# magneano/shyft

Measured on AMD Instinct MI355X. Metric: cell-steps/sec (cells×timesteps/wall) for pt_gs_k at 1/2/4/8 MI355X, higher is better.
Workload: dtype f64

## Files before the change

include/shyft_hip.h:

```cpp
#ifndef SHYFT_HIP_H
#define SHYFT_HIP_H

#include <stddef.h>
#include <stdint.h>

#ifdef __cplusplus
extern "C" {
#endif

typedef struct shyft_hip_region shyft_hip_region;

enum shyft_hip_stack {
    SHYFT_HIP_PT_GS_K = 1, SHYFT_HIP_HBV_STACK = 2, SHYFT_HIP_PT_SS_K = 3, SHYFT_HIP_PT_HS_K = 4, SHYFT_HIP_PT_HPS_K = 5
};

enum shyft_hip_forcing {
    SHYFT_HIP_TEMPERATURE = 0, SHYFT_HIP_PRECIPITATION = 1, SHYFT_HIP_WIND_SPEED = 2,
    SHYFT_HIP_REL_HUM = 3, SHYFT_HIP_RADIATION = 4
};

enum shyft_hip_collect { SHYFT_HIP_COLLECT_DISCHARGE = 0, SHYFT_HIP_COLLECT_DISCHARGE_SNOW = 1, SHYFT_HIP_COLLECT_ALL = 2 };

enum shyft_hip_ptgsk_series {
    SHYFT_HIP_AVG_DISCHARGE = 0, SHYFT_HIP_CHARGE_M3S = 1, SHYFT_HIP_SNOW_SCA = 2, SHYFT_HIP_SNOW_SWE = 3,
// ... 83 lines not shown
                         int weighted, size_t step0, size_t n, double* dst);
int shyft_hip_catchment_sums(const shyft_hip_region* h, int series, size_t step0, size_t n, double* dst,
                             int dst_on_device);
int shyft_hip_catchment_area_sums(const shyft_hip_region* h, int series, size_t step0, size_t n, double* dst,
                                  int dst_on_device);

#define SHYFT_HIP_PERCENTILES_MAX 16
#define SHYFT_HIP_PERCENTILES_LDS_MAX 4096
enum shyft_hip_statistics_property {
    SHYFT_HIP_STAT_AVERAGE = -1, SHYFT_HIP_STAT_MIN_EXTREME = -1000, SHYFT_HIP_STAT_MAX_EXTREME = 1000
};
int shyft_hip_percentiles(const shyft_hip_region* h, int series, const int64_t* ids, size_t n_ids, int scope,
                          const int64_t* pct, size_t n_pct, size_t step0, size_t n, double* dst);
int shyft_hip_catchment_percentiles(const shyft_hip_region* h, int series, const int64_t* pct, size_t n_pct,
                                    size_t step0, size_t n, double* dst, int dst_on_device);
int shyft_hip_percentiles_host(const double* rows, size_t n_steps, size_t n_samples_per_step, const int64_t* pct,
                               size_t n_pct, double* dst);
enum shyft_hip_percentiles_path_id {
    SHYFT_HIP_PERCENTILES_NONE = 0, SHYFT_HIP_PERCENTILES_LDS_SORT = 1, SHYFT_HIP_PERCENTILES_RADIX = 2
};
int shyft_hip_percentiles_path(const shyft_hip_region* h);
double shyft_hip_last_percentiles_ms(const shyft_hip_region* h);

int shyft_hip_kalman_run(int device, int n, size_t M, size_t T, const double* bias, const int32_t* fold, const double* w,
                         double v2, int mode, double* x, double* k, double* P, double* out, int save_every,
                         const int32_t* piece_begin, const int32_t* piece_ix, const double* piece_seconds);
int shyft_hip_kalman_run_host(int n, size_t M, size_t T, const double* bias, const int32_t* fold, const double* w, double v2,
                              int mode, double* x, double* k, double* P, double* out, int save_every,
                              const int32_t* piece_begin, const int32_t* piece_ix, const double* piece_seconds);
int shyft_hip_kalman_initial_state(int n, double covariance_init, double hourly_correlation, double process_noise_init,
                                   double* P, double* W);
double shyft_hip_kalman_last_ms(int device);

#define SHYFT_HIP_QM_MAX_SERIES 1024
#define SHYFT_HIP_QM_PRIOR 0
#define SHYFT_HIP_QM_QM 1
#define SHYFT_HIP_QM_BLEND 2
int shyft_hip_quantile_map(int device, size_t B, size_t T, size_t F, size_t P, const double* fc, const double* w,
                           const double* pri, const int32_t* mode, const double* interp_weight,
                           int interpolated_quantiles, double* out);
int shyft_hip_quantile_map_host(size_t B, size_t T, size_t F, size_t P, const double* fc, const double* w,
                                const double* pri, const int32_t* mode, const double* interp_weight,
                                int interpolated_quantiles, double* out);
#define SHYFT_HIP_QM_PATH_NONE 0
#define SHYFT_HIP_QM_PATH_WAVE 1
#define SHYFT_HIP_QM_PATH_GROUP 2
int shyft_hip_quantile_map_last_path(int device);
double shyft_hip_quantile_map_last_ms(int device);

#define SHYFT_HIP_RESAMPLE_AVERAGE 0
#define SHYFT_HIP_RESAMPLE_INTEGRAL 1
#define SHYFT_HIP_RESAMPLE_ACCUMULATE 2
int shyft_hip_resample(int device, int mode, size_t S, const int64_t* row, const int64_t* t, const double* v,
                       const int64_t* t_end, const int32_t* fx, int64_t ta_t0, int64_t ta_dt, size_t T, double* out);
int shyft_hip_resample_host(int device, int mode, size_t S, const int64_t* row, const int64_t* t, const double* v,
                            const int64_t* t_end, const int32_t* fx, int64_t ta_t0, int64_t ta_dt, size_t T,
                            double* out);
double shyft_hip_resample_last_ms(int device);
uint64_t shyft_hip_resample_calls(int device);
#define SHYFT_HIP_RESAMPLE_PATH_AUTO 0
#define SHYFT_HIP_RESAMPLE_PATH_DIRECT 1
#define SHYFT_HIP_RESAMPLE_PATH_TILED 2
int shyft_hip_resample_set_path(int path);
int shyft_hip_resample_last_path(int device);

int shyft_hip_ts_rating_curve(int device, size_t S, const int64_t* row, const int64_t* t, const double* v,
                              const int64_t* t_end, const int32_t* fx, size_t P, const int64_t* pack_row,
                              const int64_t* curve_t, const int64_t* curve_row, const double* seg, const int64_t* pack_of,
                              double* out);
int shyft_hip_ts_rating_curve_host(int device, size_t S, const int64_t* row, const int64_t* t, const double* v,
                                   const int64_t* t_end, const int32_t* fx, size_t P, const int64_t* pack_row,
                                   const int64_t* curve_t, const int64_t* curve_row, const double* seg,
                                   const int64_t* pack_of, double* out);
int shyft_hip_ts_ice_packing(int device, size_t S, const int64_t* row, const int64_t* t, const double* v,
                             const int64_t* t_end, const int32_t* fx, const int64_t* qrow, const int64_t* qt,
                             const int64_t* window, const double* threshold, const int32_t* policy, double* out);
int shyft_hip_ts_ice_packing_host(int device, size_t S, const int64_t* row, const int64_t* t, const double* v,
                                  const int64_t* t_end, const int32_t* fx, const int64_t* qrow, const int64_t* qt,
                                  const int64_t* window, const double* threshold, const int32_t* policy, double* out);
int shyft_hip_ts_ice_packing_recession(int device, size_t S, const int64_t* row, const int64_t* t, const double* v,
                                       const int64_t* t_end, const int32_t* fx, const double* ice,
                                       const int64_t* ice_start, const int64_t* ice_end, const double* alpha,
                                       const double* recession_minimum, double* out);
int shyft_hip_ts_ice_packing_recession_host(int device, size_t S, const int64_t* row, const int64_t* t, const double* v,
                                            const int64_t* t_end, const int32_t* fx, const double* ice,
                                            const int64_t* ice_start, const int64_t* ice_end, const double* alpha,
                                            const double* recession_minimum, double* out);
int shyft_hip_ts_min_max_fill(int device, size_t S, const int64_t* row, const int64_t* t, const double* v,
                              const int64_t* t_end, const int32_t* fx, const double* min_x, const double* max_x,
                              const int64_t* max_timespan, double* out);
int shyft_hip_ts_min_max_fill_host(int device, size_t S, const int64_t* row, const int64_t* t, const double* v,
                                   const int64_t* t_end, const int32_t* fx, const double* min_x, const double* max_x,
                                   const int64_t* max_timespan, double* out);
double shyft_hip_tsprep_last_ms(int device);
uint64_t shyft_hip_tsprep_calls(int device);

int shyft_hip_forecast_skill(int device, size_t S, const int64_t* row, const int64_t* t, const double* v,
                             const int64_t* t_end, const int32_t* fx, size_t P, const int64_t* fc_row,
                             const int64_t* fc_ix, const int64_t* obs_ix, const int64_t* t0_offset, const int64_t* dt,
                             const int64_t* n, double* ns, double* sim, double* obs);
int shyft_hip_forecast_skill_host(int device, size_t S, const int64_t* row, const int64_t* t, const double* v,
                                  const int64_t* t_end, const int32_t* fx, size_t P, const int64_t* fc_row,
                                  const int64_t* fc_ix, const int64_t* obs_ix, const int64_t* t0_offset,
                                  const int64_t* dt, const int64_t* n, double* ns, double* sim, double* obs);
double shyft_hip_forecast_skill_last_ms(int device);
uint64_t shyft_hip_forecast_skill_calls(int device);

size_t shyft_hip_number_of_catchments(const shyft_hip_region* h);
int shyft_hip_catchment_ids(const shyft_hip_region* h, int64_t* cids);

int shyft_hip_region_clone(const shyft_hip_region* src, shyft_hip_region** out);

int shyft_hip_cell_series(shyft_hip_region* h, int series, size_t cell, size_t step0, size_t n, double* buf, int write);
int shyft_hip_sample_cells(const shyft_hip_region* h, int series, const int64_t* cells, size_t n_cells, size_t step0,
                           size_t n, double* dst);

enum shyft_hip_knob {
    SHYFT_HIP_KNOB_PTGSK_INSTANCE = 1, SHYFT_HIP_KNOB_BRENT_READ_DELAY = 2,
    SHYFT_HIP_KNOB_SERIAL_SHARDS = 3,
    SHYFT_HIP_KNOB_CLONE_FAIL_AT = 4,
    SHYFT_HIP_KNOB_PERCENTILES_PATH = 5
};
int shyft_hip_set_test_knob(shyft_hip_region* h, int knob, int64_t value);

int shyft_hip_forcing_ok(const shyft_hip_region* h, int* ok);


int shyft_hip_set_routing_groups(shyft_hip_region* h, const int32_t* group_of_cell, size_t n_groups);
int shyft_hip_routing_group_sums(const shyft_hip_region* h, size_t step0, size_t n, double* dst, int dst_on_device);
int shyft_hip_route(int device, size_t n_groups, size_t T, const double* group_sums, int src_on_device,
                    const double* group_uhg, const int32_t* group_len, const int32_t* group_river, size_t n_rivers,
                    const double* river_uhg, const int32_t* river_len, const int32_t* river_downstream, size_t max_len,
                    double* local, double* upstream, double* output, int dst_on_device);

int shyft_hip_ensemble_run(shyft_hip_region* h, const double* params, size_t n_members, size_t n_per_set,
                           int start_step, int n_steps, int collect);
int shyft_hip_ensemble_sums(const shyft_hip_region* h, int series, int area_weighted, size_t step0, size_t n,
                            double* dst, int dst_on_device);
double shyft_hip_ensemble_last_ms(const shyft_hip_region* h);

int shyft_hip_math_selftest(int fn, const double* x, const double* y, size_t n, double* out);

#define SHYFT_HIP_DST_EXPLOG_INLINE 0
#define SHYFT_HIP_DST_EXPLOG_CALLS 1
#define SHYFT_HIP_DST_EXPLOG_TABLE 2
#define SHYFT_HIP_DST_POWERS 3
#define SHYFT_HIP_DST_GAMMA_LEAN 4
#define SHYFT_HIP_DST_BRENT 5
#define SHYFT_HIP_DST_BRENT_SPEC4 6
#define SHYFT_HIP_DST_BRENT_SPEC2 7
#define SHYFT_HIP_DST_SKAUGEN 8
#define SHYFT_HIP_DST_SKAUGEN_GROUP2 9
#define SHYFT_HIP_DST_SKAUGEN_GROUP4 10
int shyft_hip_device_selftest(int fn, const double* in, size_t n_in_cols, size_t n, double* out, size_t n_out_cols);

#ifdef __cplusplus
}
#endif
#endif
```

shyft_amd/csrc/device/gs_brent.h:

```cpp
#pragma once
#include <hip/hip_runtime.h>

#include "ptgsk_dev.h"
#include "gamma_lean.h"

namespace shyft_dev {

__device__ __forceinline__ double gsb_calc_q(double a, double b, double z, double lga, double eps, double ap1,
                                             const gsb_k& k, bool& ok) {
    const gamma_p_result g = gsb_gamma_pq(a, z / b, lga, eps, ap1, k, ok);
    return a * b * g.p1 + z * (1.0 - g.p);
}

__device__ __noinline__ double gs_calc_q_general(double a, double b, double z, double lga) {
    return gs_calc_q(a, b, z, lga);
}

struct gsb_f {
    double a2, b2, lga2, Q1, eps, ap1;
    bool a_ok;
    gsb_k k;
    __device__ __forceinline__ gsb_f(double z1, double a1, double b1, double a2_, double b2_, double q1, double lga2_)
        : a2(a2_), b2(b2_), lga2(lga2_) {
        Q1 = q1 == q1 ? q1 : gs_calc_q_general(a1, b1, z1, dlgamma(a1));
        k = gsb_load();
        eps = detmath::gamma_snow_policy_eps(a2);
        ap1 = a2 + 1.0;
        a_ok = a2 > 0.0;
    }
    __device__ __forceinline__ double operator()(double z) const {
        bool ok;
        double cq = gsb_calc_q(a2, b2, z, lga2, eps, ap1, k, ok);
        if (!(ok && a_ok)) cq = gs_calc_q_general(a2, b2, z, lga2);
        const double v = cq - Q1;
        return v * v;
    }
};

__device__ __forceinline__ double gs_brent_point(double z1, int k) {
    const double tolerance = 0x1p-11;
    const double golden = (double)0.3819660f;
    auto golden_step = [&](double x, double lo, double hi) {
        const double mid = (lo + hi) / 2;
        const double fract1 = tolerance * fabs(x) + tolerance / 4;
        const double d2 = (x >= mid) ? lo - x : hi - x;
        const double delta = golden * d2;
        return (fabs(delta) >= fract1) ? (x + delta) : (delta > 0 ? x + fabs(fract1) : x - fabs(fract1));
    };
    if (k == 0) return z1;
    const double u1 = golden_step(z1, 0.0, z1);
    if (k == 1) return u1;
    double lo = 0.0, hi = z1, x = z1;
    if (k == 2) {
        if (u1 >= x) lo = x; else hi = x;
        x = u1;
    } else {
        if (u1 < x) lo = u1; else hi = u1;
    }
    return golden_step(x, lo, hi);
}

struct gsb_zf {
    double z, f;
};
__device__ __noinline__ gsb_zf gs_corr_lwc_spec(double z1, double a1, double b1, double a2, double b2, double q1,
                                                double lga2, int k) {
    const gsb_f f(z1, a1, b1, a2, b2, q1, lga2);
    gsb_zf r;
    r.z = gs_brent_point(z1, k);
    r.f = f(r.z);
    return r;
}

struct gsb_memo {
    double z[4], f[4];
};

template <bool MEMO>
__device__ __forceinline__ double gs_corr_lwc_lean_t(double z1, double a1, double b1, double a2, double b2, double q1,
                                                     double lga2, const gsb_memo* memo) {
#ifdef SHYFT_ABLATE_BRENT
    return z1 * 0.5;
#endif
    const gsb_f fe(z1, a1, b1, a2, b2, q1, lga2);
    gsb_memo mm;
    if (MEMO) mm = *memo;
    auto f = [&](double z) {
        if (MEMO) {
            const long long zb = __double_as_longlong(z);
            bool hit = false;
            double r = 0.0;
#pragma unroll
            for (int i = 0; i < 4; ++i)
                if (!hit && zb == __double_as_longlong(mm.z[i])) { hit = true; r = mm.f[i]; }
            if (hit) return r;
        }
        return fe(z);
    };
    double min = 0.0, max = z1;
    const double tolerance = 0x1p-11;
    const double golden = (double)0.3819660f;
    double x, w, v, u, delta, delta2, fu, fv, fw, fx, mid, fract1, fract2;
    x = w = v = max;
    fw = fv = fx = f(x);
    delta2 = delta = 0;
    int count = 60;
    do {
        mid = (min + max) / 2;
        fract1 = tolerance * fabs(x) + tolerance / 4;
        fract2 = 2 * fract1;
        if (fabs(x - mid) <= (fract2 - (max - min) / 2)) break;
        if (fabs(delta2) > fract1) {
            double r = (x - w) * (fx - fv);
            double q = (x - v) * (fx - fw);
            double p = (x - v) * q - (x - w) * r;
            q = 2 * (q - r);
            if (q > 0) p = -p;
            q = fabs(q);
            double td = delta2;
            delta2 = delta;
            if ((fabs(p) >= fabs(q * td / 2)) || (p <= q * (min - x)) || (p >= q * (max - x))) {
                delta2 = (x >= mid) ? min - x : max - x;
                delta = golden * delta2;
            } else {
                delta = p / q;
                u = x + delta;
                if (((u - min) < fract2) || ((max - u) < fract2)) delta = (mid - x) < 0 ? -fabs(fract1) : fabs(fract1);
            }
        } else {
            delta2 = (x >= mid) ? min - x : max - x;
            delta = golden * delta2;
        }
        u = (fabs(delta) >= fract1) ? (x + delta) : (delta > 0 ? x + fabs(fract1) : x - fabs(fract1));
        fu = f(u);
        if (fu <= fx) {
            if (u >= x) min = x; else max = x;
            v = w; w = x; x = u;
            fv = fw; fw = fx; fx = fu;
        } else {
            if (u < x) min = u; else max = u;
            if ((fu <= fw) || (w == x)) {
                v = w; w = u; fv = fw; fw = fu;
            } else if ((fu <= fv) || (v == x) || (v == w)) {
                v = u; fv = fu;
            }
        }
    } while (--count);
    return x;
}

__device__ __noinline__ double gs_corr_lwc_lean(double z1, double a1, double b1, double a2, double b2, double q1,
                                                double lga2) {
    return gs_corr_lwc_lean_t<false>(z1, a1, b1, a2, b2, q1, lga2, nullptr);
}

__device__ __noinline__ double gs_corr_lwc_memo(double z1, double a1, double b1, double a2, double b2, double q1,
                                                double lga2, const gsb_memo& memo) {
    return gs_corr_lwc_lean_t<true>(z1, a1, b1, a2, b2, q1, lga2, &memo);
}

}
```

shyft_amd/csrc/kernels/ptgsk.hip:

```cpp
#include <hip/hip_runtime.h>
#include <stdint.h>
#include <stdlib.h>

#include "../device/ptgsk_dev.h"
#include "../device/gs_brent.h"
#include "../device/stream.h"
#include "../device/wave_place.h"
#include "../include_internal/kernels.h"
#include "../../../include/shyft_hip.h"

using namespace shyft_dev;

#define GS_BRENT_JOB gs_corr_lwc_lean

#ifdef SHYFT_PROF
__device__ unsigned long long g_ptgsk_prof[12];
extern "C" int shyft_ptgsk_prof_read(unsigned long long* out) {
    if (hipMemcpyFromSymbol(out, HIP_SYMBOL(g_ptgsk_prof), sizeof(g_ptgsk_prof)) != hipSuccess) return 1;
    unsigned long long z[12] = {};
    return hipMemcpyToSymbol(HIP_SYMBOL(g_ptgsk_prof), z, sizeof z) != hipSuccess;
}
#define PROF_DECL unsigned long long prof_acc[6] = {0, 0, 0, 0, 0, 0}, prof_lg = 0; unsigned long long prof_t = __builtin_amdgcn_s_memtime();
#define PROF_MARK(k) do { const unsigned long long t_ = __builtin_amdgcn_s_memtime(); prof_acc[k] += t_ - prof_t; prof_t = t_; } while (0)
#define PROF_FLUSH() do { if ((threadIdx.x & 63) == 0) { for (int k_ = 0; k_ < 6; ++k_) atomicAdd(&g_ptgsk_prof[k_], prof_acc[k_]); atomicAdd(&g_ptgsk_prof[11], prof_lg); } } while (0)
#else
#define PROF_DECL
#define PROF_MARK(k) ((void)0)
#define PROF_FLUSH() ((void)0)
#endif

namespace {

#ifndef SHYFT_PTGSK_NT
#define SHYFT_PTGSK_NT 1
#endif
constexpr bool STREAM_NT = SHYFT_PTGSK_NT != 0;

constexpr int BLOCK = 256;

#ifndef SHYFT_LB_WAVES
#define SHYFT_LB_WAVES 4
#endif

#ifndef SHYFT_PTGSK_LEAN
#define SHYFT_PTGSK_LEAN 1
#endif

constexpr int BRENT_PRIO = 3;

#ifndef SHYFT_PTGSK_LGQ
#define SHYFT_PTGSK_LGQ 1
#endif
#ifndef SHYFT_PTGSK_LGQ_NOBRENT
#define SHYFT_PTGSK_LGQ_NOBRENT 0
#endif
#ifndef SHYFT_PTGSK_LGQ_JOBLG
#define SHYFT_PTGSK_LGQ_JOBLG 1
#endif

template <bool COMPACT, bool UNIFORM, bool ENS = false, int WAVES = SHYFT_LB_WAVES, int B = BLOCK, bool SPEC = false,
          bool LEAN = false>
__global__ __launch_bounds__(B, WAVES) void ptgsk_run_kernel(const ptgsk_kargs a) {
    static_assert(COMPACT, "the Brent jobs always go through the workgroup queue");
    const int cell = blockIdx.x * blockDim.x + threadIdx.x;
    bool valid = cell < a.n_cells;
    if (valid && a.active && !a.active[cell]) valid = false;
    const int lc = valid ? cell : 0;
    const size_t N = (size_t)a.n_cells;
    const size_t NF = ENS ? (size_t)a.f_cols : N;
    const size_t fcl = ENS ? (size_t)a.fcol[lc] : (size_t)lc;
    const double* __restrict__ Pg = UNIFORM ? a.params : a.params + (size_t)a.set_ix[lc] * PTGSK_NP;
    __shared__ double lpar[UNIFORM ? PTGSK_NP : 1];
    if (UNIFORM && threadIdx.x < PTGSK_NP) lpar[threadIdx.x] = a.params[threadIdx.x];
    const double* __restrict__ P = UNIFORM ? (const double*)lpar : Pg;

    const double* __restrict__ cc = a.cellc;
    gs_cell gcell;
    gcell.forest_fraction = cc[PC_FOREST * N + lc];
    gcell.altitude = cc[PC_ALTITUDE * N + lc];
    gcell.cv2 = cc[PC_CV2 * N + lc];
    gcell.inv_cv2 = cc[PC_INV_CV2 * N + lc];
    __shared__ double lcc[11][B];
    {
        const int t = threadIdx.x;
        lcc[0][t] = gcell.forest_fraction;
        lcc[1][t] = gcell.altitude;
        lcc[2][t] = gcell.cv2;
        lcc[3][t] = gcell.inv_cv2;
        lcc[4][t] = cc[PC_GLACIER * N + lc];
        lcc[5][t] = cc[PC_SNOW_STORAGE * N + lc];
        lcc[6][t] = cc[PC_KIRCHNER_ROUTED_PREC * N + lc];
        lcc[7][t] = cc[PC_DIRECT_RESPONSE * N + lc];
        lcc[8][t] = cc[PC_AREA * N + lc];
    }
#define glacier_fraction (lcc[4][threadIdx.x])
#define snow_storage_fraction (lcc[5][threadIdx.x])
#define kirchner_routed_prec (lcc[6][threadIdx.x])
#define direct_response_fraction (lcc[7][threadIdx.x])
#define kirchner_fraction (1 - lcc[7][threadIdx.x])
#define cell_area_m2 (lcc[8][threadIdx.x])
#define glacier_area_m2 (lcc[8][threadIdx.x] * lcc[4][threadIdx.x])
#define LOAD_GCELL()                                   \
    do {                                               \
        gcell.forest_fraction = lcc[0][threadIdx.x];   \
        gcell.altitude = lcc[1][threadIdx.x];          \
        gcell.cv2 = lcc[2][threadIdx.x];               \
        gcell.inv_cv2 = lcc[3][threadIdx.x];           \
    } while (0)

    const double mmh_to_m3s_scale_factor = 1 / (3600.0 * 1000.0);

    double* __restrict__ st = a.state;
    gs_state s;
    s.albedo = st[PS_ALBEDO * N + lc];
    s.lwc = st[PS_LWC * N + lc];
    s.surface_heat = st[PS_SURFACE_HEAT * N + lc];
    s.alpha = st[PS_ALPHA * N + lc];
    s.sdc_melt_mean = st[PS_SDC_MELT_MEAN * N + lc];
    s.acc_melt = st[PS_ACC_MELT * N + lc];
    s.iso_pot_energy = st[PS_ISO_POT_ENERGY * N + lc];
    s.temp_swe = st[PS_TEMP_SWE * N + lc];
    double q = st[PS_KIRCHNER_Q * N + lc];
    lcc[9][threadIdx.x] = -1.0;
    lcc[10][threadIdx.x] = 0.0;
    constexpr bool LGQ = SHYFT_PTGSK_LGQ != 0 && B == 256 && !SPEC;
    constexpr bool JOBLG = LGQ && SHYFT_PTGSK_LGQ_JOBLG != 0;
    lgamma_cache_lds<JOBLG> lgc{lcc[9], lcc[10]};
    gs_carry carry;
    int32_t err = 0;

    const size_t TW = (size_t)a.win_len;
    const double* __restrict__ f_temp = a.forcing + (size_t)FV_TEMPERATURE * TW * NF;
    const double* __restrict__ f_prec = a.forcing + (size_t)FV_PRECIPITATION * TW * NF;
    const double* __restrict__ f_ws = a.forcing + (size_t)FV_WIND_SPEED * TW * NF;
    const double* __restrict__ f_rh = a.forcing + (size_t)FV_REL_HUM * TW * NF;
    const double* __restrict__ f_rad = a.forcing + (size_t)FV_RADIATION * TW * NF;
    double* __restrict__ R = a.resp;
    const size_t RS = TW * N;
    double* __restrict__ SS = LEAN ? nullptr : a.state_series;
    const size_t SSS = (TW + 1) * N;
    const int wed = (int)Pg[PK_WED];
    const int64_t snow_lo = (int64_t)((int)(Pg[PK_WED] * 24) - (int)(Pg[PK_NWD] * 24)) * 3600000000LL;
    const int64_t snow_hi = (int64_t)(int)(Pg[PK_WED] * 24) * 3600000000LL;

    __shared__ double jz1[B], ja1[B], jb1[B], ja2[B], jb2[B], jq1[B], jlg2[B], jres[B];
    __shared__ double jsz[SPEC ? 64 : 1], jsf[SPEC ? 64 : 1];
    __shared__ int jcount[2];
    __shared__ unsigned short lq[LGQ ? B : 1];
    __shared__ unsigned short jown[JOBLG ? B : 1];
    __shared__ int lcount[2];
    __shared__ int wsimd[B / 64];
    publish_wave_simd(wsimd);
    if (COMPACT) {
        if (threadIdx.x == 0) {
            jcount[0] = jcount[1] = 0;
            if (LGQ) lcount[0] = lcount[1] = 0;
        }
        __syncthreads();
    }
    const int jrot = solver_lane0<B>(wsimd);

    auto collect_state = [&](size_t wi) {
        SS[0 * SSS + wi * N + cell] = cell_area_m2 * q * mmh_to_m3s_scale_factor;
        SS[1 * SSS + wi * N + cell] = s.albedo;
        SS[2 * SSS + wi * N + cell] = s.lwc * snow_storage_fraction;
        SS[3 * SSS + wi * N + cell] = s.surface_heat;
        SS[4 * SSS + wi * N + cell] = s.alpha;
        SS[5 * SSS + wi * N + cell] = s.sdc_melt_mean;
        SS[6 * SSS + wi * N + cell] = s.acc_melt;
        SS[7 * SSS + wi * N + cell] = s.iso_pot_energy;
        SS[8 * SSS + wi * N + cell] = s.temp_swe * snow_storage_fraction;
    };

    const int i_end = a.step0 + a.n_steps;
    PROF_DECL
    for (int i = a.step0; i < i_end; ++i) {
        const double gm_direct = P[PK_GM_DIRECT];
        const double gm_routed = 1 - gm_direct;
        const double dtf = P[PK_DTF];
        const double p_corr = P[PK_PCORR];
        const double kc1 = P[PK_C1], kc2 = P[PK_C2], kc3 = P[PK_C3];
        const size_t wi = (size_t)(i - a.win0);
        const size_t fo = wi * N + lc;
        const size_t ff = ENS ? wi * NF + fcl : fo;
        double temp = 0, rad = 0, rel_hum = 0, prec = 0, wind_speed = 0;
        if (valid) {
            temp = stream_ld<STREAM_NT && !ENS>(&f_temp[ff]);
            rad = stream_ld<STREAM_NT && !ENS>(&f_rad[ff]);
            rel_hum = stream_ld<STREAM_NT && !ENS>(&f_rh[ff]);
            prec = stream_ld<STREAM_NT && !ENS>(&f_prec[ff]) * p_corr;
            wind_speed = stream_ld<STREAM_NT && !ENS>(&f_ws[ff]);
            if (SS) collect_state(wi);
        }
        const bool start_melt = a.doy[i] == wed;
        const int64_t trel = a.t_rel_year_us[i];
        const bool snow_season = trel >= snow_lo && trel < snow_hi;

        gs_mid m;
        m.need = false;
        m.done = true;
        LOAD_GCELL();
        if (threadIdx.x == 0) {
            jcount[(i + 1) & 1] = 0;
            if (LGQ) lcount[(i + 1) & 1] = 0;
        }
        int slot = -1;
        bool queued = false;
        auto new_shape = [&](double shape) {
            if (LGQ && shape != lcc[9][threadIdx.x]) {
                lq[atomicAdd(&lcount[i & 1], 1)] = (unsigned short)threadIdx.x;
                lcc[9][threadIdx.x] = shape;
                queued = true;
            }
        };
        auto brent_jobs = [&](int first, int nj) {
            if (JOBLG)
                for (int j = first; j < nj; j += B) {
                    const double lga2 = dlgamma(ja2[j]);
                    jlg2[j] = lga2;
                    const int o = jown[j];
                    if (lcc[9][o] == ja2[j]) lcc[10][o] = lga2;
                }
            for (int j = first; j < nj; j += B)
                jres[j] = GS_BRENT_JOB(jz1[j], ja1[j], jb1[j], ja2[j], jb2[j], jq1[j], jlg2[j]);
        };
        auto lgamma_jobs = [&](int first, int stride, int nl) {
            for (int j = first; j < nl; j += stride) {
                const int o = lq[j];
                lcc[10][o] = dlgamma(lcc[9][o]);
            }
        };
        auto enqueue = [&](double z1, double a1, double b1, double a2, double b2, double q1, double lga2) {
            slot = atomicAdd(&jcount[i & 1], 1);
            jz1[slot] = z1; ja1[slot] = a1; jb1[slot] = b1; ja2[slot] = a2; jb2[slot] = b2;
            jq1[slot] = q1; jlg2[slot] = lga2;
            if (JOBLG) jown[slot] = (unsigned short)threadIdx.x;
        };
#ifndef SHYFT_ABLATE_SNOW
        if (valid)
            gs_front(s, m, start_melt, a.dt_s, a.dt_us, P, gcell, temp, rad, prec, wind_speed, rel_hum, lgc, carry, enqueue,
                     new_shape);
#endif
        PROF_MARK(0);
        double z = 0.0;
        {
            __syncthreads();
            PROF_MARK(1);
            const int nj = jcount[i & 1];
            const int nl = LGQ ? lcount[i & 1] : 0;
            auto lgamma_phase = [&](int t) {
                const int ns = (nj + 63) & ~63;
                if (ns >= B) lgamma_jobs(t, B, nl);
                else if (t >= ns) lgamma_jobs(t - ns, B - ns, nl);
            };
            if (nj > 0) {
#ifdef SHYFT_PROF
                const unsigned long long tb = __builtin_amdgcn_s_memtime();
                if (threadIdx.x < nj) __builtin_amdgcn_s_setprio(BRENT_PRIO);
                brent_jobs((int)threadIdx.x, nj);
                __builtin_amdgcn_s_setprio(0);
                if (threadIdx.x < nj && (threadIdx.x & 63) == 0)
                    atomicAdd(&g_ptgsk_prof[8], (unsigned long long)(__builtin_amdgcn_s_memtime() - tb));
                if (LGQ && nl > 0) {
                    const unsigned long long tl = __builtin_amdgcn_s_memtime();
                    lgamma_phase((int)threadIdx.x);
                    prof_lg += __builtin_amdgcn_s_memtime() - tl;
                }
#else
                const int t = SPEC ? (int)threadIdx.x : (int)((threadIdx.x - jrot) & (B - 1));
                if (t < nj) __builtin_amdgcn_s_setprio(BRENT_PRIO);
                const int L = SPEC ? (4 * nj <= 64 ? 4 : 2 * nj <= 64 ? 2 : 0) : 0;
                if (L) {
                    const int jj = L == 4 ? t >> 2 : t >> 1;
                    if (t < 64 && jj < nj) {
                        const gsb_zf r = gs_corr_lwc_spec(jz1[jj], ja1[jj], jb1[jj], ja2[jj], jb2[jj], jq1[jj], jlg2[jj], t & (L - 1));
                        jsz[t] = r.z;
                        jsf[t] = r.f;
                    }
                    __syncthreads();
                    if (t < nj) {
                        gsb_memo mm;
#pragma unroll
                        for (int k = 0; k < 4; ++k) {
                            const int e = L * t + (k < L ? k : 0);
                            mm.z[k] = jsz[e];
                            mm.f[k] = jsf[e];
                        }
                        jres[t] = gs_corr_lwc_memo(jz1[t], ja1[t], jb1[t], ja2[t], jb2[t], jq1[t], jlg2[t], mm);
                    }
                } else {
                    brent_jobs(t, nj);
                }
                __builtin_amdgcn_s_setprio(0);
                if (LGQ && nl > 0) lgamma_phase(t);
#endif
                __syncthreads();
                if (!LEAN && a.read_delay > 0 && (threadIdx.x >> 6) != 0)
                    for (int k = 0; k < a.read_delay; ++k) __builtin_amdgcn_s_sleep(127);
                if (slot >= 0) z = jres[slot];
            } else if (LGQ && SHYFT_PTGSK_LGQ_NOBRENT > 0 && nl >= SHYFT_PTGSK_LGQ_NOBRENT) {
                lgamma_jobs((int)threadIdx.x, B, nl);
                __syncthreads();
            } else if (LGQ && queued) {
                lcc[10][threadIdx.x] = dlgamma(lcc[9][threadIdx.x]);
            }
        }
        PROF_MARK(2);
        if (!valid) {
            carry = gs_carry();
            continue;
        }
        double gs_sca, gs_storage, gs_outflow;
        LOAD_GCELL();
#ifdef SHYFT_ABLATE_SNOW
        gs_sca = 0.0; gs_storage = 0.0; gs_outflow = prec + 0.0 * z;
#else
        gs_back(s, m, z, gs_sca, gs_storage, gs_outflow, snow_season, a.dt_us, P, gcell, prec, lgc, carry);
#endif
        PROF_MARK(3);

        const double sca_area = cell_area_m2 * gs_sca;
        double gm_melt_m3s = 0.0;
        if (!(glacier_area_m2 <= sca_area || temp <= 0.0))
            gm_melt_m3s = dtf * temp * (glacier_area_m2 - sca_area) * (0.001 / 86400.0);
        double ae_exp;
        const double pot_evap =
            pt_pot_evap_exp<true>(P[PK_PT_ALBEDO], P[PK_PT_ALPHA], temp, rad, rel_hum, -q * 3.0 / P[PK_AE_SCALE], ae_exp) *
            3600.0;
        const double ae = pot_evap * (1.0 - ae_exp) * (1.0 - smax(gs_sca, glacier_fraction));
        const double gm_mmh = gm_melt_m3s / (mmh_to_m3s_scale_factor * cell_area_m2);
        PROF_MARK(4);
        double q_avg;
        if (!kirchner_step<true>(q, q_avg, gs_outflow * snow_storage_fraction + prec * kirchner_routed_prec + gm_routed * gm_mmh,
                           ae, a.t1_hours, kc1, kc2, kc3))
            err = ERR_KIRCHNER_MAX_ITER;
        const double total_discharge = smax(0.0, prec - ae) * direct_response_fraction + gm_direct * gm_mmh +
                                       q_avg * kirchner_fraction;
        const double charge_m3s = +(cell_area_m2 * prec * mmh_to_m3s_scale_factor) -
                                  (cell_area_m2 * ae * mmh_to_m3s_scale_factor) + gm_melt_m3s -
                                  (cell_area_m2 * total_discharge * mmh_to_m3s_scale_factor);
        stream_st<STREAM_NT>(&R[0 * RS + fo], cell_area_m2 * total_discharge * mmh_to_m3s_scale_factor);
        stream_st<STREAM_NT>(&R[1 * RS + fo], charge_m3s);
        if (!LEAN && a.collect >= 1) {
            R[2 * RS + fo] = gs_sca;
            R[3 * RS + fo] = gs_storage * snow_storage_fraction;
        }
        if (!LEAN && a.collect >= 2) {
            R[4 * RS + fo] = cell_area_m2 * (gs_outflow * snow_storage_fraction) * mmh_to_m3s_scale_factor;
            R[5 * RS + fo] = gm_melt_m3s;
            R[6 * RS + fo] = ae;
            R[7 * RS + fo] = pot_evap;
        }
        if (SS && i + 1 == i_end) collect_state(wi + 1);
        PROF_MARK(5);
    }
    PROF_FLUSH();
    if (!valid) return;
    st[PS_ALBEDO * N + cell] = s.albedo;
    st[PS_LWC * N + cell] = s.lwc;
    st[PS_SURFACE_HEAT * N + cell] = s.surface_heat;
    st[PS_ALPHA * N + cell] = s.alpha;
    st[PS_SDC_MELT_MEAN * N + cell] = s.sdc_melt_mean;
    st[PS_ACC_MELT * N + cell] = s.acc_melt;
    st[PS_ISO_POT_ENERGY * N + cell] = s.iso_pot_energy;
    st[PS_TEMP_SWE * N + cell] = s.temp_swe;
    st[PS_KIRCHNER_Q * N + cell] = q;
    if (err) a.err[cell] = err;
}
#undef LOAD_GCELL
#undef glacier_fraction
#undef snow_storage_fraction
#undef kirchner_routed_prec
#undef direct_response_fraction
#undef kirchner_fraction
#undef cell_area_m2
#undef glacier_area_m2

#ifndef SHYFT_PTGSK_BUDGET_WAVES
#define SHYFT_PTGSK_BUDGET_WAVES 7
#endif
__global__ __launch_bounds__(256, SHYFT_PTGSK_BUDGET_WAVES) void ptgsk_callee_budget_kernel(const ptgsk_kargs a) {
    if (a.n_cells >= 0) return;
    const int c = threadIdx.x;
    gs_state s{};
    gs_mid m{};
    lgamma_cache lgc;
    gs_carry carry;
    gs_cell gc{};
    double q = a.dt_s, qa = 0.0, sca, sto, outf;
    double j[7] = {};
    gs_front(s, m, c == 0, a.dt_s, a.dt_us, a.params, gc, q, q, q, q, q, lgc, carry,
             [&](double z1, double a1, double b1, double a2, double b2, double q1, double lga2) {
                 j[0] = z1; j[1] = a1; j[2] = b1; j[3] = a2; j[4] = b2; j[5] = q1; j[6] = lga2;
             });
    const double z = gs_corr_lwc_lean(j[0], j[1], j[2], j[3], j[4], j[5], j[6]);
    gs_back(s, m, z, sca, sto, outf, c == 1, a.dt_us, a.params, gc, q, lgc, carry);
    double e;
    const double pe = pt_pot_evap_exp<true>(0.2, 1.26, q, q, q, q, e);
    kirchner_step<true>(q, qa, outf, pe * e, a.t1_hours, -2.4, 0.9, -0.1);
    a.resp[c] = q + qa + sca + sto + s.lwc;
}

constexpr int ST_BLOCK = 256;

__global__ __launch_bounds__(ST_BLOCK, SHYFT_PTGSK_BUDGET_WAVES) void ptgsk_st_explog_inline_kernel(
    const double* __restrict__ in, size_t n, double* __restrict__ out) {
    const size_t i = blockIdx.x * (size_t)ST_BLOCK + threadIdx.x;
    if (i >= n) return;
    const kmath<true> km;
    const double x = in[i];
    out[i] = km.exp(x);
    out[n + i] = km.log(x);
}

__global__ __launch_bounds__(ST_BLOCK, SHYFT_PTGSK_BUDGET_WAVES) void ptgsk_st_explog_calls_kernel(
    const double* __restrict__ in, size_t n, double* __restrict__ out) {
    const size_t i = blockIdx.x * (size_t)ST_BLOCK + threadIdx.x;
    if (i >= n) return;
    const double x = in[i], y = in[n + i];
    out[i] = dexp(x);
    out[n + i] = dlog(x);
    const dexp_pair e = dexp2(x, y);
    out[2 * n + i] = e.a;
    out[3 * n + i] = e.b;
}

__global__ __launch_bounds__(ST_BLOCK, SHYFT_PTGSK_BUDGET_WAVES) void ptgsk_st_powers_kernel(
    const double* __restrict__ in, size_t n, double* __restrict__ out) {
    const size_t i = blockIdx.x * (size_t)ST_BLOCK + threadIdx.x;
    if (i >= n) return;
    const double x = in[i], y = in[n + i];
    out[i] = dpowr(x, y);
    out[n + i] = dpow4(x);
    out[2 * n + i] = dpow8(x);
    out[3 * n + i] = dpow(x, y);
}

__global__ __launch_bounds__(ST_BLOCK, SHYFT_PTGSK_BUDGET_WAVES) void ptgsk_st_gamma_kernel(
    const double* __restrict__ in, size_t n, double* __restrict__ out) {
    const size_t i = blockIdx.x * (size_t)ST_BLOCK + threadIdx.x;
    if (i >= n) return;
    const double a = in[i], x = in[n + i];
    const double lga = dlgamma(a);
    bool ok;
    (void)gsb_gamma_pq(a, x, lga, detmath::gamma_snow_policy_eps(a), a + 1.0, gsb_load(), ok);
    const gamma_p_result r = gs_gamma_pq_cs(a, x, lga);
    out[i] = r.p;
    out[n + i] = r.p1;
    out[2 * n + i] = r.prefix;
    out[3 * n + i] = ok ? 1.0 : 0.0;
}

__device__ __forceinline__ double st_brent_q1(double mode, double z1, double a1, double b1) {
    return mode != 0.0 ? gs_calc_q(a1, b1, z1, dlgamma(a1)) : __builtin_nan("");
}

__global__ __launch_bounds__(ST_BLOCK, SHYFT_PTGSK_BUDGET_WAVES) void ptgsk_st_brent_kernel(
    const double* __restrict__ in, size_t n, double* __restrict__ out) {
    const size_t i = blockIdx.x * (size_t)ST_BLOCK + threadIdx.x;
    if (i >= n) return;
    const double z1 = in[i], a1 = in[n + i], b1 = in[2 * n + i], a2 = in[3 * n + i], b2 = in[4 * n + i];
    const double q1 = st_brent_q1(in[5 * n + i], z1, a1, b1);
    const double lga2 = dlgamma(a2);
#ifdef SHYFT_PROF
    int nf_evals = 0;
    out[i] = gs_corr_lwc(z1, a1, b1, a2, b2, q1, lga2, nf_evals);
#else
    out[i] = gs_corr_lwc(z1, a1, b1, a2, b2, q1, lga2);
#endif
    out[n + i] = GS_BRENT_JOB(z1, a1, b1, a2, b2, q1, lga2);
}

template <int L>
__global__ __launch_bounds__(64, 2) void ptgsk_st_brent_spec_kernel(const double* __restrict__ in, size_t n,
                                                                    double* __restrict__ out) {
    static_assert(L == 4 || L == 2, "4 or 2 point lanes per job");
    constexpr int JOBS = 64 / L;
    __shared__ double jz1[JOBS], ja1[JOBS], jb1[JOBS], ja2[JOBS], jb2[JOBS], jq1[JOBS], jlg2[JOBS];
    __shared__ double jsz[64], jsf[64];
    const int t = threadIdx.x;
    const size_t j0 = blockIdx.x * (size_t)JOBS;
    const int nj = n - j0 < (size_t)JOBS ? (int)(n - j0) : JOBS;
    if (t < nj) {
        const size_t i = j0 + t;
        jz1[t] = in[i]; ja1[t] = in[n + i]; jb1[t] = in[2 * n + i]; ja2[t] = in[3 * n + i]; jb2[t] = in[4 * n + i];
        jq1[t] = st_brent_q1(in[5 * n + i], jz1[t], ja1[t], jb1[t]);
        jlg2[t] = dlgamma(ja2[t]);
    }
    __syncthreads();
    const int jj = L == 4 ? t >> 2 : t >> 1;
    if (t < 64 && jj < nj) {
        const gsb_zf r = gs_corr_lwc_spec(jz1[jj], ja1[jj], jb1[jj], ja2[jj], jb2[jj], jq1[jj], jlg2[jj], t & (L - 1));
        jsz[t] = r.z;
        jsf[t] = r.f;
    }
    __syncthreads();
    if (t < nj) {
        gsb_memo mm;
#pragma unroll
        for (int k = 0; k < 4; ++k) {
            const int e = L * t + (k < L ? k : 0);
            mm.z[k] = jsz[e];
            mm.f[k] = jsf[e];
        }
        out[j0 + t] = gs_corr_lwc_memo(jz1[t], ja1[t], jb1[t], ja2[t], jb2[t], jq1[t], jlg2[t], mm);
    }
}

}


hipError_t launch_ptgsk_run(const ptgsk_kargs& a, hipStream_t stream) {
    const int grid = (a.n_cells + BLOCK - 1) / BLOCK;
    if (grid == 0) return hipSuccess;
    int n_cu = 256;
    {
        int dev = 0;
        if (hipGetDevice(&dev) == hipSuccess) {
            int v = 0;
            if (hipDeviceGetAttribute(&v, hipDeviceAttributeMultiprocessorCount, dev) == hipSuccess && v > 0) n_cu = v;
        }
    }
    static const char* force = getenv("SHYFT_PTGSK_WAVES");
    const bool small = a.instance ? a.instance == 2 : force ? force[0] == '2' : grid <= 2 * n_cu;
    const bool lean = SHYFT_PTGSK_LEAN && a.collect == 0 && !a.state_series && a.read_delay == 0;
    if (a.n_cells < 0)
        hipLaunchKernelGGL(ptgsk_callee_budget_kernel, dim3(1), dim3(BLOCK), 0, stream, a);
    if (a.fcol) {
        hipLaunchKernelGGL((ptgsk_run_kernel<true, false, true>), dim3(grid), dim3(BLOCK), 0, stream, a);
    } else if (small) {
        const int g64 = (a.n_cells + 63) / 64;
        if (lean) {
            if (a.uniform_params) hipLaunchKernelGGL((ptgsk_run_kernel<true, true, false, 2, 64, true, true>), dim3(g64), dim3(64), 0, stream, a);
            else hipLaunchKernelGGL((ptgsk_run_kernel<true, false, false, 2, 64, true, true>), dim3(g64), dim3(64), 0, stream, a);
        } else if (a.uniform_params) hipLaunchKernelGGL((ptgsk_run_kernel<true, true, false, 2, 64, true>), dim3(g64), dim3(64), 0, stream, a);
        else hipLaunchKernelGGL((ptgsk_run_kernel<true, false, false, 2, 64, true>), dim3(g64), dim3(64), 0, stream, a);
    } else if (lean) {
        if (a.uniform_params) hipLaunchKernelGGL((ptgsk_run_kernel<true, true, false, SHYFT_LB_WAVES, BLOCK, false, true>), dim3(grid), dim3(BLOCK), 0, stream, a);
        else hipLaunchKernelGGL((ptgsk_run_kernel<true, false, false, SHYFT_LB_WAVES, BLOCK, false, true>), dim3(grid), dim3(BLOCK), 0, stream, a);
    } else {
        if (a.uniform_params) hipLaunchKernelGGL((ptgsk_run_kernel<true, true>), dim3(grid), dim3(BLOCK), 0, stream, a);
        else hipLaunchKernelGGL((ptgsk_run_kernel<true, false>), dim3(grid), dim3(BLOCK), 0, stream, a);
    }
    return hipGetLastError();
}

hipError_t launch_ptgsk_selftest(int fn, const double* in, size_t n, double* out, hipStream_t stream) {
    if (n == 0) return hipSuccess;
    const dim3 grid((unsigned)((n + ST_BLOCK - 1) / ST_BLOCK)), block(ST_BLOCK);
    switch (fn) {
        case SHYFT_HIP_DST_EXPLOG_INLINE: hipLaunchKernelGGL(ptgsk_st_explog_inline_kernel, grid, block, 0, stream, in, n, out); break;
        case SHYFT_HIP_DST_EXPLOG_CALLS: hipLaunchKernelGGL(ptgsk_st_explog_calls_kernel, grid, block, 0, stream, in, n, out); break;
        case SHYFT_HIP_DST_POWERS: hipLaunchKernelGGL(ptgsk_st_powers_kernel, grid, block, 0, stream, in, n, out); break;
        case SHYFT_HIP_DST_GAMMA_LEAN: hipLaunchKernelGGL(ptgsk_st_gamma_kernel, grid, block, 0, stream, in, n, out); break;
        case SHYFT_HIP_DST_BRENT: hipLaunchKernelGGL(ptgsk_st_brent_kernel, grid, block, 0, stream, in, n, out); break;
        case SHYFT_HIP_DST_BRENT_SPEC4:
            hipLaunchKernelGGL(ptgsk_st_brent_spec_kernel<4>, dim3((unsigned)((n + 15) / 16)), dim3(64), 0, stream, in, n, out);
            break;
        case SHYFT_HIP_DST_BRENT_SPEC2:
            hipLaunchKernelGGL(ptgsk_st_brent_spec_kernel<2>, dim3((unsigned)((n + 31) / 32)), dim3(64), 0, stream, in, n, out);
            break;
        default: return hipErrorInvalidValue;
    }
    return hipGetLastError();
}
```

shyft_amd/csrc/kernels/selftest.hip:

```cpp
#include <hip/hip_runtime.h>

#include <string>
#include <vector>

#include "../../../include/shyft_hip.h"
#include "../device/special.h"
#include "../include_internal/kernels.h"

namespace {

__global__ void math_selftest_kernel(int fn, const double* __restrict__ x, const double* __restrict__ y, size_t n,
                                     double* __restrict__ out) {
    const size_t i = blockIdx.x * (size_t)blockDim.x + threadIdx.x;
    if (i >= n) return;
    double r;
    switch (fn) {
        case 0: r = shyft_dev::dexp(x[i]); break;
        case 1: r = shyft_dev::dlog(x[i]); break;
        case 2: r = shyft_dev::dpow(x[i], y[i]); break;
        case 3: r = shyft_dev::dlgamma(x[i]); break;
        default: r = shyft_dev::gamma_p(x[i], y[i]); break;
    }
    out[i] = r;
}

}

extern "C" int shyft_hip_math_selftest(int fn, const double* x, const double* y, size_t n, double* out) {
    if (fn < 0 || fn > 4 || !x || !out || ((fn == 2 || fn == 4) && !y)) return 1;
    if (n == 0) return 0;
    double *dx = nullptr, *dy = nullptr, *dout = nullptr;
    int rc = 1;
    if (hipMalloc(&dx, n * sizeof(double)) != hipSuccess) goto done;
    if (hipMalloc(&dy, n * sizeof(double)) != hipSuccess) goto done;
    if (hipMalloc(&dout, n * sizeof(double)) != hipSuccess) goto done;
    if (hipMemcpy(dx, x, n * sizeof(double), hipMemcpyHostToDevice) != hipSuccess) goto done;
    if (y && hipMemcpy(dy, y, n * sizeof(double), hipMemcpyHostToDevice) != hipSuccess) goto done;
    hipLaunchKernelGGL(math_selftest_kernel, dim3((unsigned)((n + 255) / 256)), dim3(256), 0, 0, fn, dx, dy, n, dout);
    if (hipGetLastError() != hipSuccess) goto done;
    if (hipMemcpy(out, dout, n * sizeof(double), hipMemcpyDeviceToHost) != hipSuccess) goto done;
    rc = 0;
done:
    if (dx) (void)hipFree(dx);
    if (dy) (void)hipFree(dy);
    if (dout) (void)hipFree(dout);
    return rc;
}

extern "C" int shyft_hip_device_selftest(int fn, const double* in, size_t n_in_cols, size_t n, double* out,
                                         size_t n_out_cols) {
    static const struct { size_t n_in, n_out; bool ptssk; } spec[] = {
        {1, 2, false}, {2, 4, false}, {2, 4, true}, {2, 4, false}, {2, 4, false}, {6, 2, false},
        {6, 1, false}, {6, 1, false}, {4, 2, true}, {4, 2, true}, {4, 2, true}};
    if (fn < 0 || fn >= (int)(sizeof spec / sizeof spec[0]) || !in || !out) return 1;
    if (n_in_cols != spec[fn].n_in || n_out_cols != spec[fn].n_out) return 1;
    if (n == 0) return 0;
    double *din = nullptr, *dout = nullptr;
    int rc = 1;
    if (hipMalloc(&din, n_in_cols * n * sizeof(double)) != hipSuccess) goto done;
    if (hipMalloc(&dout, n_out_cols * n * sizeof(double)) != hipSuccess) goto done;
    if (hipMemcpy(din, in, n_in_cols * n * sizeof(double), hipMemcpyHostToDevice) != hipSuccess) goto done;
    if (hipMemset(dout, 0xff, n_out_cols * n * sizeof(double)) != hipSuccess) goto done;
    if ((spec[fn].ptssk ? launch_ptssk_selftest(fn, din, n, dout, 0) : launch_ptgsk_selftest(fn, din, n, dout, 0)) !=
        hipSuccess)
        goto done;
    if (hipDeviceSynchronize() != hipSuccess) goto done;
    if (hipMemcpy(out, dout, n_out_cols * n * sizeof(double), hipMemcpyDeviceToHost) != hipSuccess) goto done;
    rc = 0;
done:
    if (din) (void)hipFree(din);
    if (dout) (void)hipFree(dout);
    return rc;
}
```

Baseline: 11.42 billion.

## Speculatively evaluate Brent minimizer's first points across lane groups in gamma-snow jobs

Adds an open-coded Brent minimizer job in which groups of 2 or 4 lanes each evaluate one of the first deterministic golden-section points of a queued gamma-snow LWC-correction job. The results are shuffled to the group leader, which skips those function evaluations when its trajectory matches. The mode is enabled by default for the 256-thread non-spec kernel when the job queue is small (at most 16 or 32 jobs). It also merges the job arrays into a single LDS block. This trades idle lanes for fewer serial gamma evaluations per job, at the cost of extra divergence, register pressure and a new noinline call path.

```diff
diff --git a/include/shyft_hip.h b/include/shyft_hip.h
--- a/include/shyft_hip.h
+++ b/include/shyft_hip.h
@@ -259,6 +259,8 @@
 #define SHYFT_HIP_DST_SKAUGEN 8
 #define SHYFT_HIP_DST_SKAUGEN_GROUP2 9
 #define SHYFT_HIP_DST_SKAUGEN_GROUP4 10
+#define SHYFT_HIP_DST_BRENT_OPEN4 11
+#define SHYFT_HIP_DST_BRENT_OPEN2 12
 int shyft_hip_device_selftest(int fn, const double* in, size_t n_in_cols, size_t n, double* out, size_t n_out_cols);
 
 #ifdef __cplusplus
diff --git a/shyft_amd/csrc/device/gs_brent.h b/shyft_amd/csrc/device/gs_brent.h
--- a/shyft_amd/csrc/device/gs_brent.h
+++ b/shyft_amd/csrc/device/gs_brent.h
@@ -23,6 +23,13 @@
     __device__ __forceinline__ gsb_f(double z1, double a1, double b1, double a2_, double b2_, double q1, double lga2_)
         : a2(a2_), b2(b2_), lga2(lga2_) {
         Q1 = q1 == q1 ? q1 : gs_calc_q_general(a1, b1, z1, dlgamma(a1));
+        k = gsb_load();
+        eps = detmath::gamma_snow_policy_eps(a2);
+        ap1 = a2 + 1.0;
+        a_ok = a2 > 0.0;
+    }
+    __device__ __forceinline__ gsb_f(double a2_, double b2_, double lga2_, double Q1_)
+        : a2(a2_), b2(b2_), lga2(lga2_), Q1(Q1_) {
         k = gsb_load();
         eps = detmath::gamma_snow_policy_eps(a2);
         ap1 = a2 + 1.0;
@@ -159,4 +166,139 @@
     return gs_corr_lwc_lean_t<true>(z1, a1, b1, a2, b2, q1, lga2, &memo);
 }
 
-}
+enum { GSQ_Z1, GSQ_A1, GSQ_B1, GSQ_A2, GSQ_B2, GSQ_Q1, GSQ_LG2, GSQ_RES, GSQ_ROWS };
+typedef __attribute__((address_space(3))) double gsq_lds;
+
+#define GSB_NEXT_POINT(go)                                                                                          \
+    do {                                                                                                            \
+        mid = (min + max) / 2;                                                                                      \
+        fract1 = tolerance * fabs(x) + tolerance / 4;                                                               \
+        fract2 = 2 * fract1;                                                                                        \
+        go = !(fabs(x - mid) <= (fract2 - (max - min) / 2));                                                        \
+        if (!go) break;                                                                                             \
+        if (fabs(delta2) > fract1) {                                                                                \
+            double r = (x - w) * (fx - fv);                                                                         \
+            double q = (x - v) * (fx - fw);                                                                         \
+            double p = (x - v) * q - (x - w) * r;                                                                   \
+            q = 2 * (q - r);                                                                                        \
+            if (q > 0) p = -p;                                                                                      \
+            q = fabs(q);                                                                                            \
+            double td = delta2;                                                                                     \
+            delta2 = delta;                                                                                         \
+            if ((fabs(p) >= fabs(q * td / 2)) || (p <= q * (min - x)) || (p >= q * (max - x))) {                    \
+                delta2 = (x >= mid) ? min - x : max - x;                                                            \
+                delta = golden * delta2;                                                                            \
+            } else {                                                                                                \
+                delta = p / q;                                                                                      \
+                u = x + delta;                                                                                      \
+                if (((u - min) < fract2) || ((max - u) < fract2))                                                   \
+                    delta = (mid - x) < 0 ? -fabs(fract1) : fabs(fract1);                                           \
+            }                                                                                                       \
+        } else {                                                                                                    \
+            delta2 = (x >= mid) ? min - x : max - x;                                                                \
+            delta = golden * delta2;                                                                                \
+        }                                                                                                           \
+        u = (fabs(delta) >= fract1) ? (x + delta) : (delta > 0 ? x + fabs(fract1) : x - fabs(fract1));              \
+    } while (0)
+#define GSB_TAKE()                                                                                                  \
+    do {                                                                                                            \
+        if (fu <= fx) {                                                                                             \
+            if (u >= x) min = x; else max = x;                                                                      \
+            v = w; w = x; x = u;                                                                                    \
+            fv = fw; fw = fx; fx = fu;                                                                              \
+        } else {                                                                                                    \
+            if (u < x) min = u; else max = u;                                                                       \
+            if ((fu <= fw) || (w == x)) {                                                                           \
+                v = w; w = u; fv = fw; fw = fu;                                                                     \
+            } else if ((fu <= fv) || (v == x) || (v == w)) {                                                        \
+                v = u; fv = fu;                                                                                     \
+            }                                                                                                       \
+        }                                                                                                           \
+    } while (0)
+
+template <int MODE>
+__device__ __forceinline__ int gs_brent_group(int nj) {
+    return (MODE >= 1 && nj <= 16) ? 4 : (MODE >= 2 && nj <= 32) ? 2 : 1;
+}
+
+template <int B>
+__device__ __noinline__ void gs_brent_job_open(gsq_lds* jq_, int t, int L_) {
+    const int L = __builtin_amdgcn_readfirstlane(L_);
+    gsq_lds* const jq = (gsq_lds*)(uintptr_t)__builtin_amdgcn_readfirstlane((int)(uintptr_t)jq_);
+    const int j = L == 4 ? t >> 2 : L == 2 ? t >> 1 : t;
+    const double z1 = jq[GSQ_Z1 * B + j];
+#ifdef SHYFT_ABLATE_BRENT
+    if (((int)__lane_id() & (L - 1)) == 0) jq[GSQ_RES * B + j] = z1 * 0.5;
+    return;
+#endif
+    const gsb_f fe(z1, jq[GSQ_A1 * B + j], jq[GSQ_B1 * B + j], jq[GSQ_A2 * B + j], jq[GSQ_B2 * B + j],
+                   jq[GSQ_Q1 * B + j], jq[GSQ_LG2 * B + j]);
+    double min = 0.0, max = z1;
+    const double tolerance = 0x1p-11;
+    const double golden = (double)0.3819660f;
+    double x, w, v, u, delta, delta2, fu, fv, fw, fx, mid, fract1, fract2;
+    x = w = v = max;
+    delta2 = delta = 0;
+    static_assert(B <= (1 << 16), "job index field");
+    int count = (j << 8) | 60;
+    bool go = true;
+    {
+        const int lane = (int)__lane_id(), k = lane & (L - 1), g0 = lane & ~(L - 1);
+        u = gs_brent_point(z1, k);
+        fu = fe(u);
+        double sz1 = 0.0, sf1 = 0.0, sz2 = 0.0, sf2 = 0.0, sz3 = 0.0, sf3 = 0.0;
+        if (L >= 2) {
+            sz1 = __shfl(u, g0 + 1);
+            sf1 = __shfl(fu, g0 + 1);
+        }
+        if (L == 4) {
+            sz2 = __shfl(u, g0 + 2);
+            sf2 = __shfl(fu, g0 + 2);
+            sz3 = __shfl(u, g0 + 3);
+            sf3 = __shfl(fu, g0 + 3);
+        }
+        if (k != 0) return;
+        fw = fv = fx = fu;
+        if (L >= 2) do {
+            GSB_NEXT_POINT(go);
+            if (!go) break;
+            if (__double_as_longlong(u) != __double_as_longlong(sz1)) {
+                delta2 = delta = 0;
+                break;
+            }
+            fu = sf1;
+            GSB_TAKE();
+            --count;
+            if (L == 4) {
+                const double d = delta, d2 = delta2;
+                GSB_NEXT_POINT(go);
+                if (!go) break;
+                if (__double_as_longlong(u) == __double_as_longlong(sz2)) fu = sf2;
+                else if (__double_as_longlong(u) == __double_as_longlong(sz3)) fu = sf3;
+                else {
+                    delta = d;
+                    delta2 = d2;
+                    break;
+                }
+                GSB_TAKE();
+                --count;
+            }
+        } while (0);
+    }
+    if (go) do {
+        GSB_NEXT_POINT(go);
+        if (!go) break;
+        double a2o = fe.a2;
+        asm volatile("" : "+v"(a2o));
+        gsb_f fl = fe;
+        fl.ap1 = a2o + 1.0;
+        fl.eps = detmath::gamma_snow_policy_eps(a2o);
+        fu = fl(u);
+        GSB_TAKE();
+    } while (--count & 0xff);
+    jq[GSQ_RES * B + (count >> 8)] = x;
+}
+#undef GSB_NEXT_POINT
+#undef GSB_TAKE
+
+}
diff --git a/shyft_amd/csrc/kernels/ptgsk.hip b/shyft_amd/csrc/kernels/ptgsk.hip
--- a/shyft_amd/csrc/kernels/ptgsk.hip
+++ b/shyft_amd/csrc/kernels/ptgsk.hip
@@ -56,6 +56,10 @@
 #endif
 #ifndef SHYFT_PTGSK_LGQ_JOBLG
 #define SHYFT_PTGSK_LGQ_JOBLG 1
+#endif
+
+#ifndef SHYFT_PTGSK_BOPEN
+#define SHYFT_PTGSK_BOPEN 2
 #endif
 
 template <bool COMPACT, bool UNIFORM, bool ENS = false, int WAVES = SHYFT_LB_WAVES, int B = BLOCK, bool SPEC = false,
@@ -125,6 +129,7 @@
     lcc[10][threadIdx.x] = 0.0;
     constexpr bool LGQ = SHYFT_PTGSK_LGQ != 0 && B == 256 && !SPEC;
     constexpr bool JOBLG = LGQ && SHYFT_PTGSK_LGQ_JOBLG != 0;
+    constexpr int BOPEN = (B == 256 && !SPEC) ? SHYFT_PTGSK_BOPEN : 0;
     lgamma_cache_lds<JOBLG> lgc{lcc[9], lcc[10]};
     gs_carry carry;
     int32_t err = 0;
@@ -143,7 +148,17 @@
     const int64_t snow_lo = (int64_t)((int)(Pg[PK_WED] * 24) - (int)(Pg[PK_NWD] * 24)) * 3600000000LL;
     const int64_t snow_hi = (int64_t)(int)(Pg[PK_WED] * 24) * 3600000000LL;
 
-    __shared__ double jz1[B], ja1[B], jb1[B], ja2[B], jb2[B], jq1[B], jlg2[B], jres[B];
+    __shared__ double jq[SPEC ? 1 : GSQ_ROWS][SPEC ? 1 : B];
+    __shared__ double sz1[SPEC ? B : 1], sa1[SPEC ? B : 1], sb1[SPEC ? B : 1], sa2[SPEC ? B : 1], sb2[SPEC ? B : 1],
+        sq1[SPEC ? B : 1], slg2[SPEC ? B : 1], sres[SPEC ? B : 1];
+    double* const jz1 = SPEC ? sz1 : jq[GSQ_Z1];
+    double* const ja1 = SPEC ? sa1 : jq[GSQ_A1];
+    double* const jb1 = SPEC ? sb1 : jq[GSQ_B1];
+    double* const ja2 = SPEC ? sa2 : jq[GSQ_A2];
+    double* const jb2 = SPEC ? sb2 : jq[GSQ_B2];
+    double* const jq1 = SPEC ? sq1 : jq[GSQ_Q1];
+    double* const jlg2 = SPEC ? slg2 : jq[GSQ_LG2];
+    double* const jres = SPEC ? sres : jq[GSQ_RES];
     __shared__ double jsz[SPEC ? 64 : 1], jsf[SPEC ? 64 : 1];
     __shared__ int jcount[2];
     __shared__ unsigned short lq[LGQ ? B : 1];
@@ -213,15 +228,21 @@
                 queued = true;
             }
         };
-        auto brent_jobs = [&](int first, int nj) {
+        auto brent_jobs = [&](int t, int nj) {
             if (JOBLG)
-                for (int j = first; j < nj; j += B) {
+                for (int j = t; j < nj; j += B) {
                     const double lga2 = dlgamma(ja2[j]);
                     jlg2[j] = lga2;
                     const int o = jown[j];
                     if (lcc[9][o] == ja2[j]) lcc[10][o] = lga2;
                 }
-            for (int j = first; j < nj; j += B)
+            if (BOPEN) {
+                __builtin_amdgcn_fence(__ATOMIC_ACQ_REL, "wavefront");
+                const int L = gs_brent_group<BOPEN>(nj);
+                for (int tt = t; tt < L * nj; tt += B) gs_brent_job_open<B>((gsq_lds*)&jq[0][0], tt, L);
+                return;
+            }
+            for (int j = t; j < nj; j += B)
                 jres[j] = GS_BRENT_JOB(jz1[j], ja1[j], jb1[j], ja2[j], jb2[j], jq1[j], jlg2[j]);
         };
         auto lgamma_jobs = [&](int first, int stride, int nl) {
@@ -379,6 +400,7 @@
 #ifndef SHYFT_PTGSK_BUDGET_WAVES
 #define SHYFT_PTGSK_BUDGET_WAVES 7
 #endif
+constexpr int ST_BOPEN = SHYFT_PTGSK_BOPEN ? SHYFT_PTGSK_BOPEN : 2;
 __global__ __launch_bounds__(256, SHYFT_PTGSK_BUDGET_WAVES) void ptgsk_callee_budget_kernel(const ptgsk_kargs a) {
     if (a.n_cells >= 0) return;
     const int c = threadIdx.x;
@@ -393,7 +415,11 @@
              [&](double z1, double a1, double b1, double a2, double b2, double q1, double lga2) {
                  j[0] = z1; j[1] = a1; j[2] = b1; j[3] = a2; j[4] = b2; j[5] = q1; j[6] = lga2;
              });
-    const double z = gs_corr_lwc_lean(j[0], j[1], j[2], j[3], j[4], j[5], j[6]);
+    double z = gs_corr_lwc_lean(j[0], j[1], j[2], j[3], j[4], j[5], j[6]);
+    __shared__ double jq[GSQ_ROWS][BLOCK];
+    for (int r = 0; r < 7; ++r) jq[r][c] = j[r];
+    gs_brent_job_open<BLOCK>((gsq_lds*)&jq[0][0], c, 4);
+    z += jq[GSQ_RES][c];
     gs_back(s, m, z, sca, sto, outf, c == 1, a.dt_us, a.params, gc, q, lgc, carry);
     double e;
     const double pe = pt_pot_evap_exp<true>(0.2, 1.26, q, q, q, q, e);
@@ -505,6 +531,28 @@
         }
         out[j0 + t] = gs_corr_lwc_memo(jz1[t], ja1[t], jb1[t], ja2[t], jb2[t], jq1[t], jlg2[t], mm);
     }
+}
+
+template <int JOBS>
+__global__ __launch_bounds__(ST_BLOCK, SHYFT_PTGSK_BUDGET_WAVES) void ptgsk_st_brent_open_kernel(
+    const double* __restrict__ in, size_t n, double* __restrict__ out) {
+    static_assert(JOBS == 16 || JOBS == 32, "16 or 32 jobs per workgroup");
+    __shared__ double jq[GSQ_ROWS][ST_BLOCK];
+    const int t = threadIdx.x;
+    const size_t j0 = blockIdx.x * (size_t)JOBS;
+    const int nj = n - j0 < (size_t)JOBS ? (int)(n - j0) : JOBS;
+    if (t < nj) {
+        const size_t i = j0 + t;
+        jq[GSQ_Z1][t] = in[i]; jq[GSQ_A1][t] = in[n + i]; jq[GSQ_B1][t] = in[2 * n + i];
+        jq[GSQ_A2][t] = in[3 * n + i]; jq[GSQ_B2][t] = in[4 * n + i];
+        jq[GSQ_Q1][t] = st_brent_q1(in[5 * n + i], jq[GSQ_Z1][t], jq[GSQ_A1][t], jq[GSQ_B1][t]);
+        jq[GSQ_LG2][t] = dlgamma(jq[GSQ_A2][t]);
+    }
+    __syncthreads();
+    const int L = gs_brent_group<ST_BOPEN>(nj);
+    if (t < L * nj) gs_brent_job_open<ST_BLOCK>((gsq_lds*)&jq[0][0], t, L);
+    __syncthreads();
+    if (t < nj) out[j0 + t] = jq[GSQ_RES][t];
 }
 
 }
@@ -560,6 +608,12 @@
         case SHYFT_HIP_DST_BRENT_SPEC2:
             hipLaunchKernelGGL(ptgsk_st_brent_spec_kernel<2>, dim3((unsigned)((n + 31) / 32)), dim3(64), 0, stream, in, n, out);
             break;
+        case SHYFT_HIP_DST_BRENT_OPEN4:
+            hipLaunchKernelGGL(ptgsk_st_brent_open_kernel<16>, dim3((unsigned)((n + 15) / 16)), block, 0, stream, in, n, out);
+            break;
+        case SHYFT_HIP_DST_BRENT_OPEN2:
+            hipLaunchKernelGGL(ptgsk_st_brent_open_kernel<32>, dim3((unsigned)((n + 31) / 32)), block, 0, stream, in, n, out);
+            break;
         default: return hipErrorInvalidValue;
     }
     return hipGetLastError();
diff --git a/shyft_amd/csrc/kernels/selftest.hip b/shyft_amd/csrc/kernels/selftest.hip
--- a/shyft_amd/csrc/kernels/selftest.hip
+++ b/shyft_amd/csrc/kernels/selftest.hip
@@ -51,7 +51,7 @@
                                          size_t n_out_cols) {
     static const struct { size_t n_in, n_out; bool ptssk; } spec[] = {
         {1, 2, false}, {2, 4, false}, {2, 4, true}, {2, 4, false}, {2, 4, false}, {6, 2, false},
-        {6, 1, false}, {6, 1, false}, {4, 2, true}, {4, 2, true}, {4, 2, true}};
+        {6, 1, false}, {6, 1, false}, {4, 2, true}, {4, 2, true}, {4, 2, true}, {6, 1, false}, {6, 1, false}};
     if (fn < 0 || fn >= (int)(sizeof spec / sizeof spec[0]) || !in || !out) return 1;
     if (n_in_cols != spec[fn].n_in || n_out_cols != spec[fn].n_out) return 1;
     if (n == 0) return 0;
```

After: 11.66 billion, median of 6. +2.1%, better.
